# lukecq1231/nats

Measured on AMD Instinct MI355X. Metric: train_tokens_per_sec, higher is better.
Workload: dtype bf16; 1 GPU; model=distraction-gru-seq2seq, dim=1000, dim_word=100, enc_depth=1, dim_att=100, vocab=30000, src_len=800, tgt_len=100, batch_per_gpu=20, global_batch=20, seq_len=800, optimizer=adadelta+clip100, parallelism=dp1, step_graph=False

## Files before the change

nats_amd/models/distraction.py:

```python

from collections import OrderedDict

import numpy
import torch
from torch import nn

from .. import ops
from .init import init_params, param_shapes


def default_options(**overrides):
    opts = dict(
        dim_word=100,
        dim=1000,
        dim_att=100,
        encoder="gru",
        decoder="gru_cond",
        patience=10,
        max_epochs=5000,
        finish_after=10000000,
        dispFreq=100,
        decay_c=0.0,
        clip_c=-1.0,
        lrate=0.01,
        n_words=100000,
        maxlen=100,
        optimizer="adadelta",
        batch_size=16,
        valid_batch_size=16,
        saveto="model.npz",
        validFreq=1000,
        saveFreq=1000,
        sampleFreq=100,
        datasets=[],
        valid_datasets=[],
        dictionary="",
        use_dropout=False,
        reload_=False,
        verbose=False,
        enc_depth=1,
    )
    opts.update(overrides)
    return opts


class NatsModel(nn.Module):

    def __init__(self, options, params=None, seed=None):
        super().__init__()
        self.options = dict(options)
        if params is None:
            params = init_params(self.options, seed=seed)
        self.P = nn.ParameterDict()
        for k, shape in param_shapes(self.options):
            v = params[k]
            if isinstance(v, numpy.ndarray):
                t = torch.from_numpy(numpy.ascontiguousarray(v))
            else:
                t = torch.as_tensor(v)
            assert tuple(t.shape) == tuple(shape), (k, tuple(t.shape), shape)
            self.P[k] = nn.Parameter(t)

    def get_params(self):
        out = OrderedDict()
        for k, _ in param_shapes(self.options):
            out[k] = self.P[k].detach().cpu().float().numpy()
        return out

    def set_params(self, params, strict=False):
        import warnings
        with torch.no_grad():
            for k in self.P:
                if k not in params:
                    if strict:
                        raise KeyError(k)
                    warnings.warn("%s is not in the archive" % k)
                    continue
                self.P[k].copy_(torch.as_tensor(
                    numpy.ascontiguousarray(params[k]), dtype=self.P[k].dtype))

    def embed(self, ids, shift=False):
        return ops.embed_gather(self.P["Wemb"], ids, shift=shift)

    def encode(self, x, x_mask=None):
        P = self.P
        emb = self.embed(x)
        maskr = x_mask.flip(0) if x_mask is not None else None

        def bi_layer(inp, pf, pr):
            inpr = inp.flip(0)
            xg = inp @ P[pf + "_W"] + P[pf + "_b"]
            xc = inp @ P[pf + "_Wx"] + P[pf + "_bx"]
            xgr = inpr @ P[pr + "_W"] + P[pr + "_b"]
            xcr = inpr @ P[pr + "_Wx"] + P[pr + "_bx"]
            proj, projr = ops.gru_scan_bidir(
                xg, xc, x_mask, P[pf + "_U"], P[pf + "_Ux"],
                xgr, xcr, maskr, P[pr + "_U"], P[pr + "_Ux"])
            return torch.cat([proj, projr.flip(0)], dim=-1)

        ctx = bi_layer(emb, "encoder", "encoder_r")
        for l in range(1, self.options.get("enc_depth", 1)):
            ctx = bi_layer(ctx, "encoder_l%d" % l, "encoder_r_l%d" % l)
        if x_mask is not None:
            ctx_mean = ((ctx * x_mask.unsqueeze(-1)).sum(0) /
                        x_mask.sum(0).unsqueeze(-1))
        else:
            ctx_mean = ctx.mean(0)
        init_state = torch.tanh(ctx_mean @ self.P["ff_state_W"] +
                                self.P["ff_state_b"])
        return ctx, init_state

    def project_ctx(self, ctx):
        return ctx @ self.P["decoder_Wc_att"] + self.P["decoder_b_att"]

    def _dec_inputs(self, emb):
        P = self.P
        yg = emb @ P["decoder_W"] + P["decoder_b"]
        yc = emb @ P["decoder_Wx"] + P["decoder_bx"]
        return yg, yc

    def readout_logits(self, h, emb, ctxs):
        P = self.P
        logit = torch.tanh(h @ P["ff_logit_lstm_W"] + P["ff_logit_lstm_b"] +
                           emb @ P["ff_logit_prev_W"] + P["ff_logit_prev_b"] +
                           ctxs @ P["ff_logit_ctx_W"] + P["ff_logit_ctx_b"])
        return logit @ P["ff_logit_W"] + P["ff_logit_b"]

    def forward(self, x, x_mask, y, y_mask):
        ctx, init_state = self.encode(x, x_mask)
        pctx = self.project_ctx(ctx)

        emb_shifted = self.embed(y, shift=True)
        yg, yc = self._dec_inputs(emb_shifted)

        h2s, ctxs, alphas, _, _ = ops.cond_gru_scan(
            yg, yc, y_mask, init_state, ctx, x_mask, pctx, self.P)

        logits = self.readout_logits(h2s, emb_shifted, ctxs)
        T, B, V = logits.shape
        cost = ops.softmax_xent(logits.reshape(T * B, V), y.reshape(-1))
        cost = cost.reshape(T, B)
        return (cost * y_mask).sum(0)

    @torch.no_grad()
    def f_init(self, x, x_mask=None):
        ctx, init_state = self.encode(x, x_mask)
        return init_state, ctx

    @torch.no_grad()
    def f_next(self, y_prev, ctx, ctx_mask, pctx, state, acc_ctx, acc_alpha,
               generator=None, sample_draw=True):
        emb = self.embed(y_prev.clamp_min(0))
        emb = torch.where((y_prev < 0).unsqueeze(1), torch.zeros_like(emb), emb)
        yg, yc = self._dec_inputs(emb)
        h2, ctx_t, alpha_t, acc_ctx, acc_alpha = ops.cond_gru_step(
            state, yg, yc, ctx, ctx_mask, pctx, acc_ctx, acc_alpha, self.P)
        logits = self.readout_logits(h2, emb, ctx_t)
        probs = torch.softmax(logits.float(), dim=-1)
        if not sample_draw:
            sample = probs.argmax(dim=-1)
        elif generator is not None:
            sample = torch.multinomial(probs, 1, generator=generator).squeeze(1)
        else:
            sample = torch.multinomial(probs, 1).squeeze(1)
        return probs, sample, h2, alpha_t, ctx_t, acc_ctx, acc_alpha
```

nats_amd/ops/__init__.py:

```python

import os

import torch

from . import eager

_HIP = None
_HIP_TRIED = False


def _hip_ext():
    global _HIP, _HIP_TRIED
    if not _HIP_TRIED:
        _HIP_TRIED = True
        try:
            from . import hip_ext as m
            _HIP = m.load()
        except Exception:
            _HIP = None
    return _HIP


def _use_hip(*tensors):
    if os.environ.get("NATS_AMD_FORCE_EAGER"):
# ... 43 lines not shown
def _opt_slice(t, a, b, dim):
    return None if t is None else t.narrow(dim, a, b - a)


def _run_chunks(call, B, cat_dims, concurrent):
    chunks = _batch_chunks(B)
    if concurrent:
        cur = torch.cuda.current_stream()
        streams = _chunk_streams(cur.device, len(chunks))
        outs = []
        for (a, b), s in zip(chunks, streams):
            s.wait_stream(cur)
            with torch.cuda.stream(s):
                outs.append(call(a, b))
        for s in streams:
            cur.wait_stream(s)
        for o in outs:
            for t in o:
                t.record_stream(cur)
    else:
        outs = [call(a, b) for a, b in chunks]
    return tuple(torch.cat([o[i] for o in outs], dim=d)
                 for i, d in enumerate(cat_dims))


def gru_scan(x_gates, x_cand, mask, U, Ux, h0=None):
    if _use_hip(x_gates, U):
        from .gru import gru_scan_hip
        B = x_gates.shape[1]
        if B <= MAX_KERNEL_BATCH:
            return gru_scan_hip(x_gates, x_cand, mask, U, Ux, h0)
        return _run_chunks(lambda a, b: (gru_scan_hip(
            x_gates[:, a:b], x_cand[:, a:b], _opt_slice(mask, a, b, 1), U, Ux,
            _opt_slice(h0, a, b, 0)),), B, (1,), concurrent=False)[0]
    return eager.gru_scan(x_gates, x_cand, mask, U, Ux, h0)


def gru_scan_bidir(xg0, xc0, mask0, U0, Ux0, xg1, xc1, mask1, U1, Ux1):
    if _use_hip(xg0, U0):
        from .gru import gru_scan_bidir_hip
        B = xg0.shape[1]
        direct_max = MAX_KERNEL_BATCH
        if _hip_ext().gru_persistent_ok(U0.shape[0], 2 * MAX_KERNEL_BATCH):
            direct_max = 2 * MAX_KERNEL_BATCH
        if B <= direct_max:
            return gru_scan_bidir_hip(xg0, xc0, mask0, U0, Ux0, xg1, xc1,
                                      mask1, U1, Ux1)
        return _run_chunks(lambda a, b: gru_scan_bidir_hip(
            xg0[:, a:b], xc0[:, a:b], _opt_slice(mask0, a, b, 1), U0, Ux0,
            xg1[:, a:b], xc1[:, a:b], _opt_slice(mask1, a, b, 1), U1, Ux1),
            B, (1, 1), concurrent=False)
    return (eager.gru_scan(xg0, xc0, mask0, U0, Ux0),
            eager.gru_scan(xg1, xc1, mask1, U1, Ux1))


def cond_gru_scan(y_gates, y_cand, mask, init_state, ctx, ctx_mask, pctx, P):
    if _use_hip(y_gates, ctx):
        from .cond_gru import cond_gru_scan_hip
        B = y_gates.shape[1]
        if B <= MAX_KERNEL_BATCH:
            return cond_gru_scan_hip(y_gates, y_cand, mask, init_state, ctx,
                                     ctx_mask, pctx, P)
        return _run_chunks(lambda a, b: cond_gru_scan_hip(
            y_gates[:, a:b], y_cand[:, a:b], _opt_slice(mask, a, b, 1),
            init_state[a:b], ctx[:, a:b], _opt_slice(ctx_mask, a, b, 1),
            pctx[:, a:b], P), B, (1, 1, 1, 0, 0), concurrent=True)
    return eager.cond_gru_scan(y_gates, y_cand, mask, init_state, ctx,
                               ctx_mask, pctx, P)


def cond_gru_step(h_prev, x_g, x_c, ctx, ctx_mask, pctx, acc_ctx, acc_alpha, P):
    if _use_hip(h_prev, ctx):
        from .cond_gru import cond_gru_step_hip
        B = h_prev.shape[0]
        if B <= MAX_KERNEL_BATCH:
            return cond_gru_step_hip(h_prev, x_g, x_c, ctx, ctx_mask, pctx,
                                     acc_ctx, acc_alpha, P)
        return _run_chunks(lambda a, b: cond_gru_step_hip(
            h_prev[a:b], x_g[a:b], x_c[a:b], ctx[:, a:b],
            _opt_slice(ctx_mask, a, b, 1), pctx[:, a:b], acc_ctx[a:b],
            acc_alpha[a:b], P), B, (0,) * 5, concurrent=True)
    return eager.cond_gru_step(h_prev, x_g, x_c, ctx, ctx_mask, pctx,
                               acc_ctx, acc_alpha, P)


def embed_gather(Wemb, ids, shift=False):
    if (Wemb.dtype == torch.float32
            and not os.environ.get("NATS_EMBED_EAGER")
            and _use_hip(Wemb)):
        from .embed import embed_gather_hip
        return embed_gather_hip(Wemb, ids, shift=shift)
    emb = Wemb[ids.clamp_min(0)]
    if shift and ids.dim() == 2:
        shifted = torch.zeros_like(emb)
        shifted[1:] = emb[:-1]
        return shifted
    return emb


BEAM_SELECT_MAX_K = 32


def _host_ints(t):
    if not torch.is_tensor(t):
        return [int(v) for v in t]
    if t.dtype != torch.int32 or t.dim() != 1:
        raise TypeError("beam_select: seg_off and want must be 1-d int32, "
                        "got %s %s" % (t.dtype, tuple(t.shape)))
    return None if t.is_cuda else t.tolist()


def beam_select(probs, prev_cost, seg_off, want, penalty=None, use_unk=True,
                K=None):
    if probs.dim() != 2 or probs.dtype != torch.float32:
        raise TypeError("beam_select: probs must be (R, V) float32, got %s %s"
                        % (probs.dtype, tuple(probs.shape)))
    R, V = probs.shape
    for name, t in (("prev_cost", prev_cost), ("penalty", penalty)):
        if t is not None and (t.dtype != torch.float32 or t.shape != (R,)):
            raise TypeError("beam_select: %s must be (R,) float32, got %s %s"
                            % (name, t.dtype, tuple(t.shape)))
    offs, wants = _host_ints(seg_off), _host_ints(want)
    S = len(want)
    if len(seg_off) != S + 1 or S < 1:
        raise ValueError("beam_select: seg_off must have len(want)+1 entries")
    if K is None:
        if wants is None:
            raise ValueError("beam_select: pass K=max(want) when want is a "
                             "device tensor (deriving it would sync)")
        K = max(wants)
    K = int(K)
    if K > BEAM_SELECT_MAX_K:
        raise ValueError("beam_select: K=%d exceeds the kernel's %d winners "
                         "per sentence" % (K, BEAM_SELECT_MAX_K))
    if offs is not None:
        if offs[0] != 0 or offs[-1] != R:
            raise ValueError("beam_select: seg_off must run from 0 to R=%d"
                             % R)
        for s in range(S):
            live = offs[s + 1] - offs[s]
            if live < 0 or live * V >= 2 ** 31:
                raise ValueError("beam_select: sentence %d has %d x %d "
                                 "candidates; the flat index needs live*V "
                                 "in [0, 2**31)" % (s, live, V))
    if wants is not None:
        for s in range(S):
            if not 1 <= wants[s] <= K:
                raise ValueError("beam_select: want[%d]=%d outside [1, K=%d]"
                                 % (s, wants[s], K))
            if offs is not None and wants[s] > (offs[s + 1] - offs[s]) * V:
                raise ValueError("beam_select: want[%d]=%d exceeds the "
                                 "sentence's %d candidates" % (
                                     s, wants[s],
                                     (offs[s + 1] - offs[s]) * V))
    if not probs.is_contiguous():
        raise ValueError("beam_select: probs must be contiguous (row stride "
                         "V)")
    if _use_hip(probs):
        if offs is not None and wants is not None:
            tab = torch.tensor(offs + wants, dtype=torch.int32).to(
                probs.device, non_blocking=True)
            seg_off, want = tab[:S + 1], tab[S + 1:]
        else:
            seg_off = torch.as_tensor(seg_off, dtype=torch.int32,
                                      device=probs.device)
            want = torch.as_tensor(want, dtype=torch.int32,
# ... 21 lines not shown
```

nats_amd/ops/cond_gru.py:

```python

import torch

from . import _hip_ext
from . import weights_version
from .gru import (JB, _ceil, _load_opt, _pad_to, _save_opt, gru_weight_grads,
                  pack_bwd_weights, pack_fwd_weights)


def _pack_rows(mat, out_rows, out_cols):
    if mat.is_cuda and mat.dtype == torch.float32:
        ext = _hip_ext()
        if ext is not None:
            if mat.dim() == 2 and not mat.is_contiguous() and                     mat.t().is_contiguous():
                return ext.pack_pad(mat.t(), out_rows, out_cols, True)
            return ext.pack_pad(mat.contiguous(), out_rows, out_cols, False)
    return _pad_to(mat, out_rows, out_cols).to(torch.bfloat16).contiguous()


def pack_gru1_weights(U_1, W_1, Ux_1, Wx_1, Hpad, Cpad):
    if U_1.is_cuda and U_1.dtype == torch.float32:
        ext = _hip_ext()
        if ext is not None:
            return ext.pack_gru1_weights(U_1, W_1, Ux_1, Wx_1, Hpad, Cpad)
    H = Ux_1.shape[0]
# ... 43 lines not shown
                W_att, U_att, c_att, W_con, U_con, D_wei,
                acc_ctx0=None, acc_alpha0=None):
        ext = _hip_ext()
        yg = yg.to(torch.bfloat16).contiguous()
        yc = yc.to(torch.bfloat16).contiguous()
        ctx_bf = ctx.to(torch.bfloat16).contiguous()
        pctx_f = pctx.float().contiguous()
        outs = ext.cond_gru_fwd(
            yg, yc, mask, init_state, ctx_bf, ctx_mask, pctx_f,
            *pack_decoder_fwd(U, Ux, U_1, W_1, b_1, Wx_1, Ux_1, bx_1, W_att,
                              U_att, c_att, W_con, U_con, D_wei),
            acc_ctx0, acc_alpha0)
        (h2_all, ctxs_all, alphas_all, accC, accA, h1_all, saved2, saved1,
         pstate_all, ctxpre_all, accA_used, accC_used) = outs
        fctx.save_for_backward(
            yc, h1_all, h2_all, ctxs_all, alphas_all, saved2, saved1,
            pstate_all, ctxpre_all, accA_used, accC_used, ctx_bf, pctx_f,
            init_state, _save_opt(mask), U, Ux, U_1, W_1, Wx_1, Ux_1, bx_1,
            W_att, U_att, D_wei, W_con, U_con)
        fctx.in_dtypes = (yg.dtype, ctx.dtype, pctx.dtype, init_state.dtype)
        return h2_all, ctxs_all, alphas_all, accC, accA

    @staticmethod
    def backward(fctx, dh2_all, dctxs_all, dalphas_all, daccC_f, daccA_f):
        ext = _hip_ext()
        (yc, h1_all, h2_all, ctxs_all, alphas_all, saved2, saved1,
         pstate_all, ctxpre_all, accA_used, accC_used, ctx_bf, pctx_f,
         init_state, mask, U, Ux, U_1, W_1, Wx_1, Ux_1, bx_1, W_att, U_att,
         D_wei, W_con, U_con) = fctx.saved_tensors
        mask = _load_opt(mask)
        T, B, H = h2_all.shape
        C = ctx_bf.shape[2]
        A = U_att.shape[0]
        U1cat = pack_bwd_weights(U_1.float(), Ux_1.float())
        U2cat = pack_bwd_weights(U.float(), Ux.float())
        K3Hpad = U1cat.shape[1]
        if W_1.is_cuda:
            W1cat = ext.pack_cat2(W_1.float(), Wx_1.float(),
                                  _ceil(C, 16), K3Hpad)
        else:
            W1cat = _pack_rows(
                torch.cat([W_1.float(), Wx_1.float()], dim=1),
                _ceil(C, 16), K3Hpad)
        Apad32 = _ceil(A, 32)
        WattB = _pack_rows(W_att.float(), _ceil(H, 16), Apad32)

        outs = ext.cond_gru_bwd(
            dh2_all.contiguous().float(), dctxs_all, dalphas_all, daccC_f,
            daccA_f, yc, h1_all, h2_all, ctxs_all, alphas_all, saved2, saved1,
            pstate_all, ctxpre_all, accA_used, accC_used, ctx_bf, pctx_f,
            init_state, mask, U1cat, W1cat, U2cat, WattB,
            bx_1.float().contiguous(),
            D_wei.float().reshape(-1).contiguous(),
            U_att.float().reshape(-1).contiguous(),
            U_con.float().reshape(-1).contiguous(),
            W_con.float().reshape(-1).contiguous())
        (dpre1_all, dpre2_all, dctxpre_all, gdUcon, dpstate_all,
         dpctx_acc, gdDwei, gdUatt, gdcatt, dh_carry, daccC, daccA,
         gdWcon) = outs

        TB = T * B
        h1f = h1_all.reshape(TB, H).to(torch.bfloat16)
        dpr2u2 = dpre1_all[..., :2 * H].reshape(TB, 2 * H)
        dpx2 = dpre1_all[..., 2 * H:3 * H].reshape(TB, H)
        dpxa = dpre1_all[..., 3 * H:].reshape(TB, H)
        dU_1 = (h1f.t() @ dpr2u2).float()
        dUx_1 = (h1f.t() @ dpxa).float()
        ctxsf = ctxs_all.reshape(TB, C).to(torch.bfloat16)
        dW_1 = (ctxsf.t() @ dpr2u2).float()
        dWx_1 = (ctxsf.t() @ dpx2).float()
        db_1 = dpr2u2.float().sum(0)
        dbx_1 = dpxa.float().sum(0)
        dW_att = (h1f.t() @
                  dpstate_all.reshape(TB, A).to(torch.bfloat16)).float()

        dU_con = gdUcon.reshape(C, 1)
        dW_con = gdWcon.reshape(C, 1)

        dyg = dpre2_all[..., :2 * H]
        dyc = dpre2_all[..., 2 * H:3 * H]
        dU, dUx = gru_weight_grads(h2_all, dpre2_all, init_state)

        dctx_enc = torch.einsum(
            "tbs,tbc->sbc", alphas_all.to(torch.bfloat16),
            dctxpre_all).float()

        ygd, ctxd, pctxd, initd = fctx.in_dtypes
        return (dyg.to(ygd), dyc.to(ygd), None, dh_carry.to(initd),
                dctx_enc.to(ctxd), None, dpctx_acc.to(pctxd),
                dU, dUx, dU_1, dW_1, db_1, dWx_1, dUx_1, dbx_1, dW_att,
                gdUatt.reshape(A, 1), gdcatt.reshape(1),
                dW_con, dU_con, gdDwei.reshape(1, A), None, None)


def cond_gru_scan_hip(y_gates, y_cand, mask, init_state, ctx, ctx_mask, pctx,
                      P):
    if mask is not None:
        mask = mask.float().contiguous()
    if ctx_mask is not None:
        ctx_mask = ctx_mask.float().contiguous()
    return CondGRUScanFn.apply(y_gates, y_cand, mask, init_state, ctx,
                               ctx_mask, pctx, *[P[k] for k in DECODER_KEYS],
                               None, None)


def _step_packed(P):
    params = [P[k] for k in DECODER_KEYS]
    vers = weights_version(params)
    cached = getattr(P, "_nats_step_pack", None)
    if cached is not None and cached[0] == vers:
        return cached[1]
    packed = pack_decoder_fwd(*params)
    try:
        P._nats_step_pack = (vers, packed)
    except Exception:
        pass
    return packed


@torch.no_grad()
def cond_gru_step_hip(h_prev, x_g, x_c, ctx, ctx_mask, pctx, acc_ctx,
                      acc_alpha, P):
    ext = _hip_ext()
    packed = _step_packed(P)
    outs = ext.cond_gru_fwd(
        x_g.unsqueeze(0).to(torch.bfloat16).contiguous(),
        x_c.unsqueeze(0).to(torch.bfloat16).contiguous(),
        None, h_prev, ctx.to(torch.bfloat16).contiguous(),
        ctx_mask.float().contiguous() if ctx_mask is not None else None,
        pctx.float().contiguous(), *packed,
        acc_ctx.float().contiguous(), acc_alpha.float().contiguous())
    h2_all, ctxs_all, alphas_all, accC, accA = outs[:5]
    return h2_all[0], ctxs_all[0], alphas_all[0], accC, accA
```

nats_amd/ops/eager.py:

```python

import math

import torch


def gru_scan(x_gates, x_cand, mask, U, Ux, h0=None):
    T, B = x_gates.shape[0], x_gates.shape[1]
    H = Ux.shape[1]
    h = h0 if h0 is not None else x_gates.new_zeros(B, H)
    out = []
    for t in range(T):
        preact = torch.sigmoid(h @ U + x_gates[t])
        r, u = preact[:, :H], preact[:, H:]
        hbar = torch.tanh((h @ Ux) * r + x_cand[t])
        h_new = u * h + (1.0 - u) * hbar
        if mask is not None:
            m = mask[t].unsqueeze(1)
            h_new = m * h_new + (1.0 - m) * h
        h = h_new
        out.append(h)
    return torch.stack(out, dim=0)


def _attention(h1, ctx, ctx_mask, pctx, acc_ctx, acc_alpha, P):
    pstate = h1 @ P["decoder_W_att"]
    pc = pctx + pstate.unsqueeze(0)
    pc = pc + acc_alpha.t().unsqueeze(-1) * P["decoder_D_wei"].reshape(-1)
    pc = torch.tanh(pc)
    e = (pc @ P["decoder_U_att"]).squeeze(-1) + P["decoder_c_att"]
    e = e - e.max(dim=0, keepdim=True).values
    alpha = torch.exp(e)
    if ctx_mask is not None:
        alpha = alpha * ctx_mask
    alpha = alpha / alpha.sum(dim=0, keepdim=True)
    ctx_t = (ctx * alpha.unsqueeze(-1)).sum(dim=0)
    ctx_t = torch.tanh(P["decoder_U_con"].reshape(-1) * ctx_t +
                       acc_ctx * P["decoder_W_con"].reshape(-1))
    return alpha, ctx_t


def cond_gru_step(h_prev, x_g, x_c, ctx, ctx_mask, pctx, acc_ctx, acc_alpha,
                  P, m=None):
    H = h_prev.shape[1]
    preact1 = torch.sigmoid(h_prev @ P["decoder_U"] + x_g)
    r1, u1 = preact1[:, :H], preact1[:, H:]
    h1 = torch.tanh((h_prev @ P["decoder_Ux"]) * r1 + x_c)
    h1 = u1 * h_prev + (1.0 - u1) * h1
    if m is not None:
        mm = m.unsqueeze(1)
        h1 = mm * h1 + (1.0 - mm) * h_prev

    alpha, ctx_t = _attention(h1, ctx, ctx_mask, pctx, acc_ctx, acc_alpha, P)

    preact2 = torch.sigmoid(h1 @ P["decoder_U_1"] + P["decoder_b_1"] +
                            ctx_t @ P["decoder_W_1"])
    r2, u2 = preact2[:, :H], preact2[:, H:]
    h2 = torch.tanh((h1 @ P["decoder_Ux_1"] + P["decoder_bx_1"]) * r2 +
                    ctx_t @ P["decoder_Wx_1"])
    h2 = u2 * h1 + (1.0 - u2) * h2
    if m is not None:
        h2 = mm * h2 + (1.0 - mm) * h1

    if m is not None:
        new_acc_ctx = mm * ctx_t + acc_ctx
        new_acc_alpha = mm * alpha.t() + acc_alpha
    else:
        new_acc_ctx = ctx_t + acc_ctx
        new_acc_alpha = alpha.t() + acc_alpha
    return h2, ctx_t, alpha.t(), new_acc_ctx, new_acc_alpha


def cond_gru_scan(y_gates, y_cand, mask, init_state, ctx, ctx_mask, pctx, P):
    T, B = y_gates.shape[0], y_gates.shape[1]
    Ts = ctx.shape[0]
    C = ctx.shape[2]
    h = init_state
    acc_ctx = ctx.new_zeros(B, C)
    acc_alpha = ctx.new_zeros(B, Ts)
    h2s, ctxs, alphas = [], [], []
    for t in range(T):
        m = mask[t] if mask is not None else None
        h, ctx_t, alpha_t, acc_ctx, acc_alpha = cond_gru_step(
            h, y_gates[t], y_cand[t], ctx, ctx_mask, pctx, acc_ctx, acc_alpha,
            P, m=m)
        h2s.append(h)
        ctxs.append(ctx_t)
        alphas.append(alpha_t)
    return (torch.stack(h2s, 0), torch.stack(ctxs, 0), torch.stack(alphas, 0),
            acc_ctx, acc_alpha)


def softmax_xent(logits, targets):
    if logits.dtype != torch.float64:
        logits = logits.float()
    logp = torch.log_softmax(logits, dim=-1)
    return -logp.gather(1, targets.unsqueeze(1)).squeeze(1)


NEG_UNK = math.log(1e-20)


def beam_select(probs, prev_cost, seg_off, want, penalty=None, use_unk=True,
                K=None):
    offs = [int(v) for v in (seg_off.tolist() if torch.is_tensor(seg_off)
                             else seg_off)]
    wants = [int(v) for v in (want.tolist() if torch.is_tensor(want)
                              else want)]
    S = len(wants)
    K = max(wants) if K is None else int(K)
    logp = probs.log()
    if not use_unk:
        logp[:, 1] = NEG_UNK
    cand = prev_cost[:, None] - logp
    key = cand if penalty is None else cand + penalty[:, None]
    ranks = torch.full((S, K), -1, dtype=torch.int64, device=probs.device)
    costs = torch.full((S, K), float("inf"), dtype=probs.dtype,
                       device=probs.device)
    for s in range(S):
        sl = slice(offs[s], offs[s + 1])
        order = torch.sort(key[sl].flatten(), stable=True).indices[:wants[s]]
        ranks[s, :wants[s]] = order
        costs[s, :wants[s]] = cand[sl].flatten()[order]
    return ranks, costs


def rerank_penalties(hist_a, hist_c, hist_s, cur_a, cur_c, cur_s,
                     kl_factor, ctx_factor, state_factor):
    p = hist_a / hist_a.sum(-1, keepdim=True)
    q = (cur_a / cur_a.sum(-1, keepdim=True)).unsqueeze(0)
    logterm = torch.where(p > 0, p * (torch.log(p) - torch.log(q)),
                          torch.zeros_like(p))
    a_pen = -kl_factor * logterm.sum(-1).min(dim=0).values

    def cosd(h, c):
        num = (h * c.unsqueeze(0)).sum(-1)
        den = h.norm(dim=-1) * c.norm(dim=-1).unsqueeze(0)
        d = 1.0 - num / den
        return torch.where(den == 0, torch.zeros_like(d), d)

    c_pen = ctx_factor * cosd(hist_c, cur_c).max(dim=0).values
    s_pen = state_factor * cosd(hist_s, cur_s).max(dim=0).values
    return a_pen + c_pen + s_pen


def rerank_advance(anc_old, anc_new, parent, n):
    parent = torch.as_tensor(parent, dtype=torch.int64,
                             device=anc_old.device)
    R = parent.shape[0]
    anc_new[:n - 1, :R] = anc_old[:n - 1].index_select(1, parent)
    anc_new[n - 1, :R] = parent.to(anc_new.dtype)
    return anc_new


def rerank_gather(hist, anc, n, R):
    steps = torch.arange(n, device=hist.device)[:, None]
    return hist[steps, anc[:n, :R].long()]


def rerank_penalties_paged(hist_a, hist_c, hist_s, anc, n, cur_a, cur_c,
                           cur_s, kl_factor, ctx_factor, state_factor):
    R = cur_a.shape[0]
    if n == 0:
        return torch.zeros(R, dtype=cur_a.dtype, device=cur_a.device)
    return rerank_penalties(
        rerank_gather(hist_a, anc, n, R), rerank_gather(hist_c, anc, n, R),
        rerank_gather(hist_s, anc, n, R), cur_a, cur_c, cur_s,
        kl_factor, ctx_factor, state_factor)
```

nats_amd/ops/hip/bind.cpp:

```cpp

#include <torch/extension.h>

std::vector<torch::Tensor> gru_scan_fwd(torch::Tensor xg, torch::Tensor xc,
                                        c10::optional<torch::Tensor> mask,
                                        torch::Tensor Upk,
                                        c10::optional<torch::Tensor> h0);
std::vector<torch::Tensor> gru_scan_bwd(torch::Tensor dh_out,
                                        torch::Tensor h_all,
                                        torch::Tensor saved, torch::Tensor xc,
                                        c10::optional<torch::Tensor> mask,
                                        torch::Tensor Ubwd,
                                        c10::optional<torch::Tensor> h0);
std::vector<torch::Tensor> gru_scan_fwd_bidir(
    torch::Tensor xg0, torch::Tensor xc0, c10::optional<torch::Tensor> mask0,
    torch::Tensor Upk0, torch::Tensor xg1, torch::Tensor xc1,
    c10::optional<torch::Tensor> mask1, torch::Tensor Upk1);
std::vector<torch::Tensor> gru_scan_bwd_bidir(
    torch::Tensor dh_out0, torch::Tensor h_all0, torch::Tensor saved0,
    torch::Tensor xc0, c10::optional<torch::Tensor> mask0,
    torch::Tensor Ubwd0, torch::Tensor dh_out1, torch::Tensor h_all1,
    torch::Tensor saved1, torch::Tensor xc1,
    c10::optional<torch::Tensor> mask1, torch::Tensor Ubwd1);
std::vector<torch::Tensor> softmax_ce_fwd(torch::Tensor logits,
                                          torch::Tensor targets);
torch::Tensor softmax_ce_bwd(torch::Tensor logits, torch::Tensor targets,
                             torch::Tensor stats, torch::Tensor dnll);
torch::Tensor mfma_gemm_bt(torch::Tensor A, torch::Tensor Bt);
double barrier_bench(int nwg_x, int nwg_y, int iters);
bool gru_persistent_ok(long H, long B);
double barrier_bench_xcd(int nwg, int nxcd, int iters);
torch::Tensor rerank_penalties(torch::Tensor hist_a, torch::Tensor hist_c,
                               torch::Tensor hist_s, torch::Tensor cur_a,
                               torch::Tensor cur_c, torch::Tensor cur_s,
                               double kl_f, double ctx_f, double state_f);
void rerank_advance(torch::Tensor anc_old, torch::Tensor anc_new,
                    torch::Tensor parent, long n);
torch::Tensor rerank_penalties_paged(torch::Tensor hist_a,
                                     torch::Tensor hist_c,
                                     torch::Tensor hist_s, torch::Tensor anc,
                                     long n, torch::Tensor cur_a,
                                     torch::Tensor cur_c, torch::Tensor cur_s,
                                     double kl_f, double ctx_f,
                                     double state_f);
std::vector<torch::Tensor> beam_select(torch::Tensor probs,
                                       torch::Tensor prev_cost,
                                       torch::Tensor seg_off,
                                       torch::Tensor want,
                                       c10::optional<torch::Tensor> penalty,
                                       long K, bool use_unk, double neg_unk);
void fused_adadelta_step(torch::Tensor ptrs, torch::Tensor sizes,
                         torch::Tensor chunk_tensor, torch::Tensor chunk_off,
                         torch::Tensor g2, double clip_c, double rho,
                         double eps);
std::vector<torch::Tensor> cond_gru_fwd(
    torch::Tensor yg, torch::Tensor yc, c10::optional<torch::Tensor> mask,
    torch::Tensor init_state, torch::Tensor ctx_bf,
    c10::optional<torch::Tensor> ctx_mask, torch::Tensor pctx,
    torch::Tensor Upk2, torch::Tensor W1pk, torch::Tensor WattPk,
    torch::Tensor b1, torch::Tensor bx1, torch::Tensor Uatt,
    torch::Tensor catt, torch::Tensor Dwei, torch::Tensor Wcon,
    torch::Tensor Ucon,
    c10::optional<torch::Tensor> accC0, c10::optional<torch::Tensor> accA0);
std::vector<torch::Tensor> cond_gru_bwd(
    torch::Tensor dh2_all, c10::optional<torch::Tensor> dctxs_all,
    c10::optional<torch::Tensor> dalphas_all,
    c10::optional<torch::Tensor> daccC_f, c10::optional<torch::Tensor> daccA_f,
    torch::Tensor yc, torch::Tensor h1_all, torch::Tensor h2_all,
    torch::Tensor ctxs_all, torch::Tensor alphas_all, torch::Tensor saved2,
    torch::Tensor saved1, torch::Tensor pstate_all, torch::Tensor ctxpre_all,
    torch::Tensor accA_used, torch::Tensor accC_used, torch::Tensor ctx_bf,
    torch::Tensor pctx, torch::Tensor init_state,
    c10::optional<torch::Tensor> mask, torch::Tensor U1cat,
    torch::Tensor W1cat, torch::Tensor U2cat, torch::Tensor WattB,
    torch::Tensor bx1, torch::Tensor Dwei, torch::Tensor Uatt,
    torch::Tensor Ucon, torch::Tensor Wcon);

torch::Tensor embed_gather(torch::Tensor Wemb, torch::Tensor ids,
                           long shift_rows);
torch::Tensor pack_fwd_weights_hip(torch::Tensor U, torch::Tensor Ux);
torch::Tensor pack_cat2_hip(torch::Tensor A, torch::Tensor B, long R, long K);
torch::Tensor pack_pad_hip(torch::Tensor src, long R, long K, bool transpose);
torch::Tensor pack_gru1_weights_hip(torch::Tensor U_1, torch::Tensor W_1,
                                    torch::Tensor Ux_1, torch::Tensor Wx_1,
                                    long Hpad, long Cpad);
torch::Tensor embed_scatter_add(torch::Tensor dout, torch::Tensor ids,
                                long V, long shift_rows);

PYBIND11_MODULE(TORCH_EXTENSION_NAME, m) {
  m.def("pack_fwd_weights", &pack_fwd_weights_hip,
        "fused forward-scan weight pack");
  m.def("pack_cat2", &pack_cat2_hip, "fused [A|B] zero-padded bf16 pack");
  m.def("pack_pad", &pack_pad_hip, "fused pad(+transpose) bf16 pack");
  m.def("pack_gru1_weights", &pack_gru1_weights_hip,
        "fused GRU_1 4-group operand pack");
  m.def("embed_gather", &embed_gather,
        "embedding gather (+fused decoder shift)");
  m.def("embed_scatter_add", &embed_scatter_add,
        "embedding backward scatter-add");
  m.def("gru_scan_fwd", &gru_scan_fwd, "fused GRU scan forward");
  m.def("gru_scan_bwd", &gru_scan_bwd, "fused GRU scan backward");
  m.def("gru_scan_fwd_bidir", &gru_scan_fwd_bidir,
        "bidirectional fused GRU scan forward");
  m.def("gru_scan_bwd_bidir", &gru_scan_bwd_bidir,
        "bidirectional fused GRU scan backward");
  m.def("softmax_ce_fwd", &softmax_ce_fwd, "fused softmax+CE forward");
  m.def("softmax_ce_bwd", &softmax_ce_bwd, "fused softmax+CE backward");
  m.def("mfma_gemm_bt", &mfma_gemm_bt, "MFMA layout self-test GEMM");
  m.def("barrier_bench", &barrier_bench, "grid barrier us/iteration");
  m.def("gru_persistent_ok", &gru_persistent_ok,
        "persistent scan available for this hidden size and batch");
  m.def("barrier_bench_xcd", &barrier_bench_xcd,
        "XCD-constrained grid barrier us/iteration");
  m.def("rerank_penalties", &rerank_penalties,
        "fused decode-time distraction rerank reductions");
  m.def("rerank_advance", &rerank_advance,
        "ancestor-table reshuffle of the paged rerank histories");
  m.def("rerank_penalties_paged", &rerank_penalties_paged,
        "rerank reductions over slab histories read through the ancestor "
        "table (partial pass + combine pass)");
  m.def("beam_select", &beam_select,
        "segmented beam candidate selection (tile pass + merge pass)");
  m.def("fused_adadelta_step", &fused_adadelta_step,
        "fused multi-tensor global-norm clip + adadelta");
  m.def("cond_gru_fwd", &cond_gru_fwd, "fused cond-GRU decoder forward");
  m.def("cond_gru_bwd", &cond_gru_bwd, "fused cond-GRU decoder backward");
}
```

nats_amd/ops/hip/build_ext.py:

```python

import os

HERE = os.path.dirname(os.path.abspath(__file__))
BUILD_DIR = os.path.join(HERE, "build")

SOURCES = [
    os.path.join(HERE, "bind.cpp"),
    os.path.join(HERE, "gru_scan.hip"),
    os.path.join(HERE, "cond_gru.hip"),
    os.path.join(HERE, "barrier_bench.hip"),
    os.path.join(HERE, "softmax_ce.hip"),
    os.path.join(HERE, "mfma_test.hip"),
    os.path.join(HERE, "optim.hip"),
    os.path.join(HERE, "rerank.hip"),
    os.path.join(HERE, "beam_select.hip"),
    os.path.join(HERE, "embed.hip"),
    os.path.join(HERE, "pack.hip"),
]


def build(verbose=False):
    os.environ.setdefault("PYTORCH_ROCM_ARCH", "gfx950")
    os.makedirs(BUILD_DIR, exist_ok=True)
    from torch.utils.cpp_extension import load
    mod = load(
        name="nats_amd_hip",
        sources=SOURCES,
        build_directory=BUILD_DIR,
        extra_cflags=["-O3"],
        extra_cuda_cflags=["-O3", "-std=c++17"],
        verbose=verbose,
        with_cuda=True,
    )
    return mod


if __name__ == "__main__":
    build(verbose=True)
    print("built:", os.listdir(BUILD_DIR))
```

Measured before the change: 513,300 tokens/s.

## Fuse bias-add/cast into linear layers and encoder context head with custom HIP kernels

Adds a bf16 linear-with-bias autograd function whose bias add and cast run in one in-place kernel, with a fixed-order column-sum kernel for the bias gradient. The encoder's concat/flip, context mean and attention projection are fused into an encoder-head op, whose backward writes gradients straight into the forward and reverse scan dh tensors. The decoder's encoder-context gradient einsum also stays in bf16 instead of upcasting. The aim is to cut the elementwise launches and fp32 round-trips around the GEMMs, at the cost of more custom code and slightly different rounding in the bias and context gradients.

```diff
diff --git a/nats_amd/models/distraction.py b/nats_amd/models/distraction.py
--- a/nats_amd/models/distraction.py
+++ b/nats_amd/models/distraction.py
@@ -82,53 +82,63 @@
     def embed(self, ids, shift=False):
         return ops.embed_gather(self.P["Wemb"], ids, shift=shift)
 
-    def encode(self, x, x_mask=None):
+    def _encode_scans(self, x, x_mask):
         P = self.P
         emb = self.embed(x)
         maskr = x_mask.flip(0) if x_mask is not None else None
 
         def bi_layer(inp, pf, pr):
             inpr = inp.flip(0)
-            xg = inp @ P[pf + "_W"] + P[pf + "_b"]
-            xc = inp @ P[pf + "_Wx"] + P[pf + "_bx"]
-            xgr = inpr @ P[pr + "_W"] + P[pr + "_b"]
-            xcr = inpr @ P[pr + "_Wx"] + P[pr + "_bx"]
-            proj, projr = ops.gru_scan_bidir(
+            xg = ops.linear_bias(inp, P[pf + "_W"], P[pf + "_b"])
+            xc = ops.linear_bias(inp, P[pf + "_Wx"], P[pf + "_bx"])
+            xgr = ops.linear_bias(inpr, P[pr + "_W"], P[pr + "_b"])
+            xcr = ops.linear_bias(inpr, P[pr + "_Wx"], P[pr + "_bx"])
+            return ops.gru_scan_bidir(
                 xg, xc, x_mask, P[pf + "_U"], P[pf + "_Ux"],
                 xgr, xcr, maskr, P[pr + "_U"], P[pr + "_Ux"])
-            return torch.cat([proj, projr.flip(0)], dim=-1)
 
-        ctx = bi_layer(emb, "encoder", "encoder_r")
+        proj, projr = bi_layer(emb, "encoder", "encoder_r")
         for l in range(1, self.options.get("enc_depth", 1)):
-            ctx = bi_layer(ctx, "encoder_l%d" % l, "encoder_r_l%d" % l)
-        if x_mask is not None:
-            ctx_mean = ((ctx * x_mask.unsqueeze(-1)).sum(0) /
-                        x_mask.sum(0).unsqueeze(-1))
-        else:
-            ctx_mean = ctx.mean(0)
-        init_state = torch.tanh(ctx_mean @ self.P["ff_state_W"] +
-                                self.P["ff_state_b"])
-        return ctx, init_state
+            ctx = torch.cat([proj, projr.flip(0)], dim=-1)
+            proj, projr = bi_layer(ctx, "encoder_l%d" % l,
+                                   "encoder_r_l%d" % l)
+        return proj, projr
+
+    def _init_state(self, ctx_mean):
+        return torch.tanh(ctx_mean @ self.P["ff_state_W"] +
+                          self.P["ff_state_b"])
+
+    def encode(self, x, x_mask=None):
+        proj, projr = self._encode_scans(x, x_mask)
+        ctx = torch.cat([proj, projr.flip(0)], dim=-1)
+        return ctx, self._init_state(ops.eager.context_mean(ctx, x_mask))
 
     def project_ctx(self, ctx):
         return ctx @ self.P["decoder_Wc_att"] + self.P["decoder_b_att"]
 
     def _dec_inputs(self, emb):
         P = self.P
-        yg = emb @ P["decoder_W"] + P["decoder_b"]
-        yc = emb @ P["decoder_Wx"] + P["decoder_bx"]
+        yg = ops.linear_bias(emb, P["decoder_W"], P["decoder_b"])
+        yc = ops.linear_bias(emb, P["decoder_Wx"], P["decoder_bx"])
         return yg, yc
+
+    def _readout_hidden(self, h, emb, ctxs):
+        P = self.P
+        return torch.tanh(h @ P["ff_logit_lstm_W"] + P["ff_logit_lstm_b"] +
+                          emb @ P["ff_logit_prev_W"] + P["ff_logit_prev_b"] +
+                          ctxs @ P["ff_logit_ctx_W"] + P["ff_logit_ctx_b"])
 
     def readout_logits(self, h, emb, ctxs):
         P = self.P
-        logit = torch.tanh(h @ P["ff_logit_lstm_W"] + P["ff_logit_lstm_b"] +
-                           emb @ P["ff_logit_prev_W"] + P["ff_logit_prev_b"] +
-                           ctxs @ P["ff_logit_ctx_W"] + P["ff_logit_ctx_b"])
+        logit = self._readout_hidden(h, emb, ctxs)
         return logit @ P["ff_logit_W"] + P["ff_logit_b"]
 
     def forward(self, x, x_mask, y, y_mask):
-        ctx, init_state = self.encode(x, x_mask)
-        pctx = self.project_ctx(ctx)
+        P = self.P
+        proj, projr = self._encode_scans(x, x_mask)
+        ctx, ctx_mean, pctx = ops.encoder_head(
+            proj, projr, x_mask, P["decoder_Wc_att"], P["decoder_b_att"])
+        init_state = self._init_state(ctx_mean)
 
         emb_shifted = self.embed(y, shift=True)
         yg, yc = self._dec_inputs(emb_shifted)
@@ -136,7 +146,8 @@
         h2s, ctxs, alphas, _, _ = ops.cond_gru_scan(
             yg, yc, y_mask, init_state, ctx, x_mask, pctx, self.P)
 
-        logits = self.readout_logits(h2s, emb_shifted, ctxs)
+        logits = ops.linear_bias(self._readout_hidden(h2s, emb_shifted, ctxs),
+                                 P["ff_logit_W"], P["ff_logit_b"])
         T, B, V = logits.shape
         cost = ops.softmax_xent(logits.reshape(T * B, V), y.reshape(-1))
         cost = cost.reshape(T, B)
diff --git a/nats_amd/ops/__init__.py b/nats_amd/ops/__init__.py
--- a/nats_amd/ops/__init__.py
+++ b/nats_amd/ops/__init__.py
@@ -149,6 +149,25 @@
             acc_alpha[a:b], P), B, (0,) * 5, concurrent=True)
     return eager.cond_gru_step(h_prev, x_g, x_c, ctx, ctx_mask, pctx,
                                acc_ctx, acc_alpha, P)
+
+
+def _autocast_bf16():
+    return (torch.is_autocast_enabled("cuda")
+            and torch.get_autocast_dtype("cuda") == torch.bfloat16)
+
+
+def linear_bias(x, W, b):
+    if _use_hip(x, W) and _autocast_bf16():
+        from .io_fusion import linear_bias_hip
+        return linear_bias_hip(x, W, b)
+    return eager.linear_bias(x, W, b)
+
+
+def encoder_head(h_f, h_r, x_mask, Wc_att, b_att):
+    if _use_hip(h_f, Wc_att) and _autocast_bf16():
+        from .io_fusion import encoder_head_hip
+        return encoder_head_hip(h_f, h_r, x_mask, Wc_att, b_att)
+    return eager.encoder_head(h_f, h_r, x_mask, Wc_att, b_att)
 
 
 def embed_gather(Wemb, ids, shift=False):
diff --git a/nats_amd/ops/cond_gru.py b/nats_amd/ops/cond_gru.py
--- a/nats_amd/ops/cond_gru.py
+++ b/nats_amd/ops/cond_gru.py
@@ -149,8 +149,7 @@
         dU, dUx = gru_weight_grads(h2_all, dpre2_all, init_state)
 
         dctx_enc = torch.einsum(
-            "tbs,tbc->sbc", alphas_all.to(torch.bfloat16),
-            dctxpre_all).float()
+            "tbs,tbc->sbc", alphas_all.to(torch.bfloat16), dctxpre_all)
 
         ygd, ctxd, pctxd, initd = fctx.in_dtypes
         return (dyg.to(ygd), dyc.to(ygd), None, dh_carry.to(initd),
diff --git a/nats_amd/ops/eager.py b/nats_amd/ops/eager.py
--- a/nats_amd/ops/eager.py
+++ b/nats_amd/ops/eager.py
@@ -97,6 +97,22 @@
     return -logp.gather(1, targets.unsqueeze(1)).squeeze(1)
 
 
+def linear_bias(x, W, b):
+    return x @ W + b
+
+
+def context_mean(ctx, x_mask):
+    if x_mask is not None:
+        return ((ctx * x_mask.unsqueeze(-1)).sum(0) /
+                x_mask.sum(0).unsqueeze(-1))
+    return ctx.mean(0)
+
+
+def encoder_head(h_f, h_r, x_mask, Wc_att, b_att):
+    ctx = torch.cat([h_f, h_r.flip(0)], dim=-1)
+    return ctx, context_mean(ctx, x_mask), ctx @ Wc_att + b_att
+
+
 NEG_UNK = math.log(1e-20)
 
 
diff --git a/nats_amd/ops/hip/bind.cpp b/nats_amd/ops/hip/bind.cpp
--- a/nats_amd/ops/hip/bind.cpp
+++ b/nats_amd/ops/hip/bind.cpp
@@ -85,6 +85,15 @@
                                     long Hpad, long Cpad);
 torch::Tensor embed_scatter_add(torch::Tensor dout, torch::Tensor ids,
                                 long V, long shift_rows);
+torch::Tensor bias_cast_(torch::Tensor g, torch::Tensor b);
+torch::Tensor colsum_bf16(torch::Tensor g);
+long colsum_rows_per_block();
+torch::Tensor ctx_head_fwd(torch::Tensor hf, torch::Tensor hr);
+std::vector<torch::Tensor> ctx_head_bwd(torch::Tensor denc,
+                                        torch::Tensor dproj,
+                                        torch::Tensor dmean,
+                                        c10::optional<torch::Tensor> mask,
+                                        torch::Tensor cnt);
 
 PYBIND11_MODULE(TORCH_EXTENSION_NAME, m) {
   m.def("pack_fwd_weights", &pack_fwd_weights_hip,
@@ -97,6 +106,16 @@
         "embedding gather (+fused decoder shift)");
   m.def("embed_scatter_add", &embed_scatter_add,
         "embedding backward scatter-add");
+  m.def("bias_cast_", &bias_cast_,
+        "in-place y = bf16(float(g) + b) on a bf16 GEMM result");
+  m.def("colsum_bf16", &colsum_bf16,
+        "fp32 column sums of a row-strided bf16 matrix (fixed order)");
+  m.def("colsum_rows_per_block", &colsum_rows_per_block,
+        "rows one colsum_bf16 partial block reduces");
+  m.def("ctx_head_fwd", &ctx_head_fwd,
+        "bf16 [h_f | flip(h_r)] context");
+  m.def("ctx_head_bwd", &ctx_head_bwd,
+        "context gradient terms summed into the scans' dh tensors");
   m.def("gru_scan_fwd", &gru_scan_fwd, "fused GRU scan forward");
   m.def("gru_scan_bwd", &gru_scan_bwd, "fused GRU scan backward");
   m.def("gru_scan_fwd_bidir", &gru_scan_fwd_bidir,
diff --git a/nats_amd/ops/hip/build_ext.py b/nats_amd/ops/hip/build_ext.py
--- a/nats_amd/ops/hip/build_ext.py
+++ b/nats_amd/ops/hip/build_ext.py
@@ -16,6 +16,7 @@
     os.path.join(HERE, "beam_select.hip"),
     os.path.join(HERE, "embed.hip"),
     os.path.join(HERE, "pack.hip"),
+    os.path.join(HERE, "io_fusion.hip"),
 ]
 
 
diff --git a/nats_amd/ops/hip/io_fusion.hip b/nats_amd/ops/hip/io_fusion.hip
--- /dev/null
+++ b/nats_amd/ops/hip/io_fusion.hip
@@ -0,0 +1,350 @@
+
+#include <torch/extension.h>
+#include <ATen/cuda/CUDAContext.h>
+
+#include "common.h"
+
+namespace {
+
+typedef __bf16 bf16x4 __attribute__((ext_vector_type(4)));
+
+constexpr int IO_BLOCK = 256;
+constexpr int IO_WAVES = IO_BLOCK / NATS_WAVE;
+
+constexpr int COLSUM_ROWS = 128;
+constexpr int CTX_TCHUNK = 16;
+
+inline bool aligned_to(const void* p, size_t a) {
+  return (reinterpret_cast<uintptr_t>(p) & (a - 1)) == 0;
+}
+
+inline int grid_for(long work, int per_block, int cap) {
+  long g = (work + per_block - 1) / per_block;
+  return (int)(g < 1 ? 1 : (g > cap ? cap : g));
+}
+
+
+__global__ void bias_cast_vec_kernel(bf16_t* __restrict__ g,
+                                     const float* __restrict__ b, long n8,
+                                     int N) {
+  const long stride = (long)gridDim.x * blockDim.x;
+  for (long i = (long)blockIdx.x * blockDim.x + threadIdx.x; i < n8;
+       i += stride) {
+    const int n = (int)((i * 8) % N);
+    bf16x8 v = *(const bf16x8*)(g + i * 8);
+    const f32x4 b0 = *(const f32x4*)(b + n);
+    const f32x4 b1 = *(const f32x4*)(b + n + 4);
+#pragma unroll
+    for (int j = 0; j < 4; ++j) {
+      v[j] = (bf16_t)((float)v[j] + b0[j]);
+      v[4 + j] = (bf16_t)((float)v[4 + j] + b1[j]);
+    }
+    *(bf16x8*)(g + i * 8) = v;
+  }
+}
+
+__global__ void bias_cast_scalar_kernel(bf16_t* __restrict__ g,
+                                        const float* __restrict__ b,
+                                        long total, int N) {
+  const long stride = (long)gridDim.x * blockDim.x;
+  for (long i = (long)blockIdx.x * blockDim.x + threadIdx.x; i < total;
+       i += stride)
+    g[i] = (bf16_t)((float)g[i] + b[i % N]);
+}
+
+
+template <int VEC>
+__global__ void colsum_partial_kernel(const bf16_t* __restrict__ g, long ld,
+                                      int R, int N,
+                                      float* __restrict__ part) {
+  __shared__ float red[IO_WAVES][NATS_WAVE * VEC];
+  const int lane = threadIdx.x & (NATS_WAVE - 1);
+  const int w = threadIdx.x / NATS_WAVE;
+  const int n0 = (blockIdx.x * NATS_WAVE + lane) * VEC;
+  const int r0 = blockIdx.y * COLSUM_ROWS;
+  const int r1 = min(r0 + COLSUM_ROWS, R);
+  float acc[VEC];
+#pragma unroll
+  for (int j = 0; j < VEC; ++j) acc[j] = 0.f;
+  if (n0 < N) {
+#pragma unroll 4
+    for (int r = r0 + w; r < r1; r += IO_WAVES) {
+      const bf16_t* p = g + (long)r * ld + n0;
+      if (VEC == 4) {
+        const bf16x4 v = *(const bf16x4*)p;
+#pragma unroll
+        for (int j = 0; j < VEC; ++j) acc[j] += (float)v[j];
+      } else {
+        acc[0] += (float)p[0];
+      }
+    }
+  }
+#pragma unroll
+  for (int j = 0; j < VEC; ++j) red[w][lane * VEC + j] = acc[j];
+  __syncthreads();
+  if (w == 0 && n0 < N) {
+#pragma unroll
+    for (int j = 0; j < VEC; ++j) {
+      float s = red[0][lane * VEC + j];
+      for (int k = 1; k < IO_WAVES; ++k) s += red[k][lane * VEC + j];
+      part[(long)blockIdx.y * N + n0 + j] = s;
+    }
+  }
+}
+
+__global__ void colsum_final_kernel(const float* __restrict__ part,
+                                    int nchunk, int N,
+                                    float* __restrict__ out) {
+  const int n = blockIdx.x * blockDim.x + threadIdx.x;
+  if (n >= N) return;
+  float s0 = 0.f, s1 = 0.f, s2 = 0.f, s3 = 0.f;
+  int c = 0;
+#pragma unroll 2
+  for (; c + 4 <= nchunk; c += 4) {
+    s0 += part[(long)c * N + n];
+    s1 += part[(long)(c + 1) * N + n];
+    s2 += part[(long)(c + 2) * N + n];
+    s3 += part[(long)(c + 3) * N + n];
+  }
+  if (c < nchunk) s0 += part[(long)c * N + n];
+  if (c + 1 < nchunk) s1 += part[(long)(c + 1) * N + n];
+  if (c + 2 < nchunk) s2 += part[(long)(c + 2) * N + n];
+  out[n] = (s0 + s1) + (s2 + s3);
+}
+
+
+template <int VEC>
+__global__ void ctx_head_fwd_kernel(const float* __restrict__ hf,
+                                    const float* __restrict__ hr,
+                                    bf16_t* __restrict__ ctx, int T, int B,
+                                    int H) {
+  const long BC = (long)B * 2 * H;
+  const long j = ((long)blockIdx.x * blockDim.x + threadIdx.x) * VEC;
+  if (j >= BC) return;
+  const int b = (int)(j / (2 * H));
+  const int c = (int)(j % (2 * H));
+  const bool rev = c >= H;
+  const long BH = (long)B * H;
+  const long src_off = (long)b * H + (rev ? c - H : c);
+  const float* src = rev ? hr : hf;
+  const int t0 = blockIdx.y * CTX_TCHUNK;
+  const int t1 = min(t0 + CTX_TCHUNK, T);
+#pragma unroll 4
+  for (int t = t0; t < t1; ++t) {
+    const int ts = rev ? T - 1 - t : t;
+    const float* p = src + (long)ts * BH + src_off;
+    bf16_t* o = ctx + (long)t * BC + j;
+    if (VEC == 4) {
+      const f32x4 v = *(const f32x4*)p;
+      bf16x4 q;
+#pragma unroll
+      for (int k = 0; k < VEC; ++k) q[k] = (bf16_t)v[k];
+      *(bf16x4*)o = q;
+    } else {
+      o[0] = (bf16_t)p[0];
+    }
+  }
+}
+
+template <int VEC>
+__global__ void ctx_head_bwd_kernel(const bf16_t* __restrict__ denc,
+                                    long es_t, long es_b,
+                                    const bf16_t* __restrict__ dproj,
+                                    const float* __restrict__ dmean,
+                                    const float* __restrict__ mask,
+                                    const float* __restrict__ cnt,
+                                    float* __restrict__ dhf,
+                                    float* __restrict__ dhr, int T, int B,
+                                    int H) {
+  const long BC = (long)B * 2 * H;
+  const long j = ((long)blockIdx.x * blockDim.x + threadIdx.x) * VEC;
+  if (j >= BC) return;
+  const int b = (int)(j / (2 * H));
+  const int c = (int)(j % (2 * H));
+  const bool rev = c >= H;
+  const long BH = (long)B * H;
+  const long dst_off = (long)b * H + (rev ? c - H : c);
+  float* dst = rev ? dhr : dhf;
+  const float n = cnt[b];
+  float dm[VEC];
+#pragma unroll
+  for (int k = 0; k < VEC; ++k) dm[k] = dmean[(long)b * 2 * H + c + k] / n;
+  const int t0 = blockIdx.y * CTX_TCHUNK;
+  const int t1 = min(t0 + CTX_TCHUNK, T);
+#pragma unroll 4
+  for (int t = t0; t < t1; ++t) {
+    const int td = rev ? T - 1 - t : t;
+    const float m = mask ? mask[(long)t * B + b] : 1.f;
+    const bf16_t* pe = denc + (long)t * es_t + (long)b * es_b + c;
+    const bf16_t* pp = dproj + (long)t * BC + j;
+    float* o = dst + (long)td * BH + dst_off;
+    if (VEC == 4) {
+      const bf16x4 e = *(const bf16x4*)pe;
+      const bf16x4 p = *(const bf16x4*)pp;
+      f32x4 r;
+#pragma unroll
+      for (int k = 0; k < VEC; ++k)
+        r[k] = ((float)e[k] + (float)p[k]) + m * dm[k];
+      *(f32x4*)o = r;
+    } else {
+      o[0] = ((float)pe[0] + (float)pp[0]) + m * dm[0];
+    }
+  }
+}
+
+}
+
+long colsum_rows_per_block() { return COLSUM_ROWS; }
+
+torch::Tensor bias_cast_(torch::Tensor g, torch::Tensor b) {
+  TORCH_CHECK(g.is_cuda() && g.dtype() == torch::kBFloat16 &&
+              g.is_contiguous() && g.dim() >= 1, "bias_cast_: g must be a "
+              "contiguous bf16 CUDA tensor");
+  const long N = g.size(-1);
+  TORCH_CHECK(b.is_cuda() && b.dtype() == torch::kFloat32 &&
+              b.is_contiguous() && b.dim() == 1 && b.size(0) == N,
+              "bias_cast_: b must be contiguous fp32 of g's last size");
+  const long total = g.numel();
+  if (total == 0) return g;
+  TORCH_CHECK(N < (1L << 31));
+  auto stream = at::cuda::getCurrentCUDAStream().stream();
+  bf16_t* gp = (bf16_t*)g.data_ptr();
+  const float* bp = b.data_ptr<float>();
+  if (N % 8 == 0 && aligned_to(gp, 16) && aligned_to(bp, 16)) {
+    const long n8 = total / 8;
+    hipLaunchKernelGGL(bias_cast_vec_kernel,
+                       dim3(grid_for(n8, IO_BLOCK, 256 * 16)), dim3(IO_BLOCK),
+                       0, stream, gp, bp, n8, (int)N);
+  } else {
+    hipLaunchKernelGGL(bias_cast_scalar_kernel,
+                       dim3(grid_for(total, IO_BLOCK, 256 * 16)),
+                       dim3(IO_BLOCK), 0, stream, gp, bp, total, (int)N);
+  }
+  HIP_CHECK(hipGetLastError());
+  return g;
+}
+
+torch::Tensor colsum_bf16(torch::Tensor g) {
+  TORCH_CHECK(g.is_cuda() && g.dtype() == torch::kBFloat16 && g.dim() == 2,
+              "colsum_bf16: g must be a 2-d bf16 CUDA tensor");
+  const long R = g.size(0), N = g.size(1);
+  TORCH_CHECK(N == 1 || g.stride(1) == 1,
+              "colsum_bf16: columns must be unit-stride");
+  const long ld = R > 1 ? g.stride(0) : N;
+  TORCH_CHECK(ld >= N && R < (1L << 31) && N < (1L << 31));
+  auto optsF = g.options().dtype(torch::kFloat32);
+  auto out = torch::empty({N}, optsF);
+  if (N == 0) return out;
+  if (R == 0) return out.zero_();
+  const int nchunk = cdiv((int)R, COLSUM_ROWS);
+  TORCH_CHECK(nchunk <= 65535, "colsum_bf16: too many rows");
+  auto part = torch::empty({nchunk, N}, optsF);
+  auto stream = at::cuda::getCurrentCUDAStream().stream();
+  const bf16_t* gp = (const bf16_t*)g.data_ptr();
+  if (N % 4 == 0 && ld % 4 == 0 && aligned_to(gp, 8)) {
+    hipLaunchKernelGGL(colsum_partial_kernel<4>,
+                       dim3(cdiv((int)N, NATS_WAVE * 4), nchunk),
+                       dim3(IO_BLOCK), 0, stream, gp, ld, (int)R, (int)N,
+                       part.data_ptr<float>());
+  } else {
+    hipLaunchKernelGGL(colsum_partial_kernel<1>,
+                       dim3(cdiv((int)N, NATS_WAVE), nchunk), dim3(IO_BLOCK),
+                       0, stream, gp, ld, (int)R, (int)N,
+                       part.data_ptr<float>());
+  }
+  HIP_CHECK(hipGetLastError());
+  hipLaunchKernelGGL(colsum_final_kernel, dim3(cdiv((int)N, IO_BLOCK)),
+                     dim3(IO_BLOCK), 0, stream, part.data_ptr<float>(),
+                     nchunk, (int)N, out.data_ptr<float>());
+  HIP_CHECK(hipGetLastError());
+  return out;
+}
+
+torch::Tensor ctx_head_fwd(torch::Tensor hf, torch::Tensor hr) {
+  TORCH_CHECK(hf.is_cuda() && hf.dtype() == torch::kFloat32 &&
+              hf.dim() == 3 && hf.is_contiguous(),
+              "ctx_head_fwd: h_f must be contiguous fp32 [T,B,H]");
+  TORCH_CHECK(hr.is_cuda() && hr.dtype() == torch::kFloat32 &&
+              hr.is_contiguous() && hr.sizes() == hf.sizes(),
+              "ctx_head_fwd: h_r must match h_f");
+  const long T = hf.size(0), B = hf.size(1), H = hf.size(2);
+  TORCH_CHECK(T >= 1 && B >= 1 && H >= 1);
+  const long C = 2 * H, BC = B * C;
+  const int nchunk = cdiv((int)T, CTX_TCHUNK);
+  TORCH_CHECK(nchunk <= 65535 && BC < (1L << 31));
+  auto ctx = torch::empty({T, B, C}, hf.options().dtype(torch::kBFloat16));
+  auto stream = at::cuda::getCurrentCUDAStream().stream();
+  if (H % 4 == 0) {
+    hipLaunchKernelGGL(ctx_head_fwd_kernel<4>,
+                       dim3(cdiv((int)(BC / 4), IO_BLOCK), nchunk),
+                       dim3(IO_BLOCK), 0, stream, hf.data_ptr<float>(),
+                       hr.data_ptr<float>(), (bf16_t*)ctx.data_ptr(), (int)T,
+                       (int)B, (int)H);
+  } else {
+    hipLaunchKernelGGL(ctx_head_fwd_kernel<1>,
+                       dim3(cdiv((int)BC, IO_BLOCK), nchunk), dim3(IO_BLOCK),
+                       0, stream, hf.data_ptr<float>(), hr.data_ptr<float>(),
+                       (bf16_t*)ctx.data_ptr(), (int)T, (int)B, (int)H);
+  }
+  HIP_CHECK(hipGetLastError());
+  return ctx;
+}
+
+std::vector<torch::Tensor> ctx_head_bwd(torch::Tensor denc,
+                                        torch::Tensor dproj,
+                                        torch::Tensor dmean,
+                                        c10::optional<torch::Tensor> mask,
+                                        torch::Tensor cnt) {
+  TORCH_CHECK(denc.is_cuda() && denc.dtype() == torch::kBFloat16 &&
+              denc.dim() == 3, "ctx_head_bwd: denc must be bf16 [T,B,2H]");
+  const long T = denc.size(0), B = denc.size(1), C = denc.size(2);
+  TORCH_CHECK(C % 2 == 0 && T >= 1 && B >= 1 && C >= 2);
+  const long H = C / 2;
+  if (denc.stride(2) != 1) denc = denc.contiguous();
+  TORCH_CHECK(dproj.is_cuda() && dproj.dtype() == torch::kBFloat16 &&
+              dproj.is_contiguous() && dproj.sizes() == denc.sizes(),
+              "ctx_head_bwd: dproj must be contiguous bf16 like denc");
+  TORCH_CHECK(dmean.is_cuda() && dmean.dtype() == torch::kFloat32 &&
+              dmean.is_contiguous() && dmean.dim() == 2 &&
+              dmean.size(0) == B && dmean.size(1) == C,
+              "ctx_head_bwd: dmean must be contiguous fp32 [B,2H]");
+  TORCH_CHECK(cnt.is_cuda() && cnt.dtype() == torch::kFloat32 &&
+              cnt.is_contiguous() && cnt.numel() == B);
+  const float* mp = nullptr;
+  if (mask.has_value()) {
+    TORCH_CHECK(mask->is_cuda() && mask->dtype() == torch::kFloat32 &&
+                mask->is_contiguous() && mask->dim() == 2 &&
+                mask->size(0) == T && mask->size(1) == B,
+                "ctx_head_bwd: mask must be contiguous fp32 [T,B]");
+    mp = mask->data_ptr<float>();
+  }
+  const long BC = B * C;
+  const int nchunk = cdiv((int)T, CTX_TCHUNK);
+  TORCH_CHECK(nchunk <= 65535 && BC < (1L << 31));
+  auto optsF = dmean.options();
+  auto dhf = torch::empty({T, B, H}, optsF);
+  auto dhr = torch::empty({T, B, H}, optsF);
+  const long es_t = T > 1 ? denc.stride(0) : 0;
+  const long es_b = B > 1 ? denc.stride(1) : 0;
+  const bf16_t* ep = (const bf16_t*)denc.data_ptr();
+  auto stream = at::cuda::getCurrentCUDAStream().stream();
+  if (H % 4 == 0 && es_t % 4 == 0 && es_b % 4 == 0 && aligned_to(ep, 8)) {
+    hipLaunchKernelGGL(ctx_head_bwd_kernel<4>,
+                       dim3(cdiv((int)(BC / 4), IO_BLOCK), nchunk),
+                       dim3(IO_BLOCK), 0, stream, ep, es_t, es_b,
+                       (const bf16_t*)dproj.data_ptr(),
+                       dmean.data_ptr<float>(), mp, cnt.data_ptr<float>(),
+                       dhf.data_ptr<float>(), dhr.data_ptr<float>(), (int)T,
+                       (int)B, (int)H);
+  } else {
+    hipLaunchKernelGGL(ctx_head_bwd_kernel<1>,
+                       dim3(cdiv((int)BC, IO_BLOCK), nchunk), dim3(IO_BLOCK),
+                       0, stream, ep, es_t, es_b,
+                       (const bf16_t*)dproj.data_ptr(),
+                       dmean.data_ptr<float>(), mp, cnt.data_ptr<float>(),
+                       dhf.data_ptr<float>(), dhr.data_ptr<float>(), (int)T,
+                       (int)B, (int)H);
+  }
+  HIP_CHECK(hipGetLastError());
+  return {dhf, dhr};
+}
diff --git a/nats_amd/ops/io_fusion.py b/nats_amd/ops/io_fusion.py
--- /dev/null
+++ b/nats_amd/ops/io_fusion.py
@@ -0,0 +1,84 @@
+
+import torch
+
+from . import _hip_ext, eager
+from .gru import _load_opt, _save_opt
+
+BF16 = torch.bfloat16
+
+
+class LinearBiasFn(torch.autograd.Function):
+
+    @staticmethod
+    def forward(ctx, x, W, b):
+        ext = _hip_ext()
+        K, N = W.shape
+        x2 = x.reshape(-1, K).to(BF16)
+        Wb = W.to(BF16)
+        y = ext.bias_cast_(x2 @ Wb, b.float().contiguous())
+        ctx.save_for_backward(x2, Wb)
+        ctx.x_shape, ctx.dtypes = x.shape, (x.dtype, W.dtype, b.dtype)
+        return y.view(*x.shape[:-1], N)
+
+    @staticmethod
+    def backward(ctx, dy):
+        ext = _hip_ext()
+        x2, Wb = ctx.saved_tensors
+        xd, Wd, bd = ctx.dtypes
+        N = Wb.shape[1]
+        dy2 = dy.to(BF16).reshape(-1, N)
+        if dy2.stride(1) != 1 and N > 1:
+            dy2 = dy2.contiguous()
+        db = ext.colsum_bf16(dy2)
+        dyc = dy2.contiguous()
+        dx = dW = None
+        if ctx.needs_input_grad[0]:
+            dx = (dyc @ Wb.t()).view(ctx.x_shape).to(xd)
+        if ctx.needs_input_grad[1]:
+            dW = (x2.t() @ dyc).to(Wd)
+        return dx, dW, db.to(bd)
+
+
+def linear_bias_hip(x, W, b):
+    return LinearBiasFn.apply(x, W, b)
+
+
+class EncoderHeadFn(torch.autograd.Function):
+
+    @staticmethod
+    def forward(fctx, h_f, h_r, mask, Wc_att, b_att):
+        ext = _hip_ext()
+        T, B, H = h_f.shape
+        fctx.dtypes = (h_f.dtype, h_r.dtype, Wc_att.dtype, b_att.dtype)
+        h_f, h_r = h_f.float().contiguous(), h_r.float().contiguous()
+        ctx_bf = ext.ctx_head_fwd(h_f, h_r)
+        ctx_mean = eager.context_mean(
+            torch.cat([h_f, h_r.flip(0)], dim=-1), mask)
+        cnt = (mask.sum(0) if mask is not None
+               else h_f.new_full((B,), float(T)))
+        Wb = Wc_att.to(BF16)
+        pctx = (ctx_bf.view(T * B, 2 * H) @ Wb).view(T, B, -1) + b_att
+        fctx.save_for_backward(ctx_bf, Wb, _save_opt(mask), cnt)
+        return ctx_bf, ctx_mean, pctx
+
+    @staticmethod
+    def backward(fctx, dctx, dmean, dpctx):
+        ext = _hip_ext()
+        ctx_bf, Wb, mask, cnt = fctx.saved_tensors
+        mask = _load_opt(mask)
+        T, B, C = ctx_bf.shape
+        A = Wb.shape[1]
+        hfd, hrd, Wd, bd = fctx.dtypes
+        db_att = dpctx.reshape(T * B, A).sum(0)
+        dpb = dpctx.to(BF16).reshape(T * B, A)
+        dWc = ctx_bf.view(T * B, C).t() @ dpb
+        dproj = (dpb @ Wb.t()).view(T, B, C)
+        dh_f, dh_r = ext.ctx_head_bwd(
+            dctx.to(BF16), dproj, dmean.float().contiguous(), mask, cnt)
+        return dh_f.to(hfd), dh_r.to(hrd), None, dWc.to(Wd), db_att.to(bd)
+
+
+def encoder_head_hip(h_f, h_r, x_mask, Wc_att, b_att):
+    if x_mask is not None:
+        x_mask = x_mask.float().contiguous()
+    return EncoderHeadFn.apply(h_f, h_r, x_mask, Wc_att, b_att)
```

New measurement: 531,300 tokens/s, median of 6. 3.5% higher.
